# razvanmatisan/duodiff

Measured on AMD Instinct MI355X. Metric: images/sec (whole node) DuoDiff 1000-step CelebA-64, higher is better.
Workload: dtype bf16

## Files before the change

### duodiff_amd/csrc/dev_harness.hip

```cpp
#include "../../include/duodiff.h"
#include "../../include/duodiff_dev.h"
#include "engine_state.h"
#include "launch_args.h"

#include <cstring>
#include <vector>

using namespace dd;

extern "C" {

int dd_dev_mlp(dd_ctx* c, int M, int D, int hidden, int extras, const float* x_host, const float* w1, const float* b1, const float* w2,
               const float* b2, float* xres_host, unsigned short* out_host, const float* ln_in, const float* ln_out,
               unsigned short* ln_out_host, int iters, void* stream, float* ms_out, const float* ao_host, const float* wproj,
               const float* bproj, const float* skip_host, const float* wskip, const float* bskip, const float* wqkv,
               unsigned short* qkv_out_host) {
    const bool proj = ao_host && wproj && bproj;
    const bool skp = skip_host && wskip && bskip;
    const bool qk = wqkv && qkv_out_host;
    if (qk && (!proj || !ln_out || (hidden / 32) % 2)) return DD_ERR_INVALID;
    if (proj && (!ln_in || D % 128)) return DD_ERR_INVALID;
    if (skp && (!proj || !ln_out || !ln_out_host || (hidden / 32) % 2)) return DD_ERR_INVALID;
    if (!c || !x_host || !w1 || !b1 || !w2 || !b2 || !xres_host || M < 1 || iters < 0 || extras < 0 || (extras > 0 && M % (1 + extras))) return DD_ERR_INVALID;
    if (!mlp_fused_supported(D, hidden)) return ctx_fail(c, DD_ERR_UNSUPPORTED, "fused MLP: D in {64,128,256,512}, hidden % 64 == 0");
// ... 506 lines not shown
    const AffineRow* dT = table ? dev.upload(tab.data(), tab.size() * sizeof(AffineRow)) : nullptr;
    const StepState* dS = table ? dev.upload(&st_host, sizeof(StepState)) : nullptr;
    auto once = [&]() { return launch_cache_extrapolate(dL, dP, dO, (long long)n, bf, dS, dT, table ? -1 : op, table ? __builtin_nanf("") : w, s); };
    DEV_HIP(dev, once());
    DEV_HIP(dev, hipStreamSynchronize(s));
    dev.download(out_host, dO, n_out * es);
    DEV_HIP(dev, time_launches(s, iters, once, ms_out));
    return dev.status();
}

int dd_dev_embed(dd_ctx* c, int B, int C, int S, int P, int D, int extras, int num_classes, int normalize, int generic, const float* x_img,
                 const float* w, const float* bias, const float* pos, const float* label_emb, const long long* y, const float* t_vec,
                 float t_state, const float* ln, float* x_tok_host, unsigned short* ln_frag_host, int iters, void* stream, float* ms_out) {
    if (!c || B < 1 || C < 1 || P < 1 || S < P || S % P || D < 2 || extras < 1 || extras > 2 || !x_img || !w || !bias || !pos || !x_tok_host ||
        (extras == 2 && (!label_emb || !y || num_classes < 1)) || (ln && !ln_frag_host) || iters < 0)
        return DD_ERR_INVALID;
    const int pd = C * P * P, L = extras + (S / P) * (S / P), Mp = round_up(B * L, 256);
    if (pd > 64) return ctx_fail(c, DD_ERR_UNSUPPORTED, "embed: patch_dim <= 64");
    hipStream_t s = (hipStream_t)stream;
    const std::vector<float> wt = transposed(w, D, pd);
    const size_t n_tok = ((size_t)Mp + 8) * D;
    EmbedArgs a{};
    a.B = B; a.C = C; a.S = S; a.P = P; a.D = D; a.L = L; a.extras = extras; a.num_classes = num_classes; a.normalize = normalize; a.Mp = Mp;
    a.generic = generic;
    if (ln && !embed_ln_supported(a)) return ctx_fail(c, DD_ERR_UNSUPPORTED, "embed with norm1: the MFMA kernel at patch 4, 3 channels, embed_dim 512");
    DevScope dev(c);
    a.x_img = dev.upload(x_img, (size_t)B * C * S * S * 4);
    a.wt = dev.upload(wt.data(), wt.size() * 4);
    a.bias = dev.upload(bias, (size_t)D * 4);
    a.pos = dev.upload(pos, (size_t)L * D * 4);
    if (extras == 2) { a.label_emb = dev.upload(label_emb, (size_t)num_classes * D * 4); a.y = dev.upload(y, (size_t)B * 8); }
    if (t_vec) a.t_vec = dev.upload(t_vec, (size_t)B * 4);
    a.st = dev.alloc<StepState>(sizeof(StepState));
    a.x_tok = dev.filled<float>(n_tok * 4, 0xFF);
    if (ln) {
        a.ln_g = dev.upload(ln, (size_t)2 * D * 4); a.ln_b = a.ln_g + D;
        a.ln_frag = dev.filled<bf16_t>(n_tok * 2, 0xFF);
    }
    DEV_HIP(dev, launch_set_state_float(a.st, t_state, s));
    auto once = [&]() { return launch_embed(a, s); };
    DEV_HIP(dev, once());
    DEV_HIP(dev, hipStreamSynchronize(s));
    dev.download(x_tok_host, a.x_tok, n_tok * 4);
    if (ln) dev.download(ln_frag_host, a.ln_frag, n_tok * 2);
    DEV_HIP(dev, time_launches(s, iters, once, ms_out));
    return dev.status();
}

int dd_dev_time_mlp(dd_ctx* c, int B, int D, int L, int extras, int normalize, const float* w1, const float* b1, const float* w2,
                    const float* b2, const float* pos, const float* t_vec, float t_state, float* x_tok_host, int iters, void* stream,
                    float* ms_out) {
    if (!c || B < 1 || D < 2 || extras < 1 || L < extras || !w1 || !b1 || !w2 || !b2 || !pos || !x_tok_host || iters < 0) return DD_ERR_INVALID;
    if ((size_t)5 * D * 4 > 64 * 1024) return ctx_fail(c, DD_ERR_UNSUPPORTED, "time_mlp: 5 D floats of LDS");
    hipStream_t s = (hipStream_t)stream;
    const int H4 = 4 * D;
    const std::vector<float> w1t = transposed(w1, H4, D), w2t = transposed(w2, D, H4);
    const size_t n_tok = (size_t)B * L * D;
    DevScope dev(c);
    StepState* st = dev.alloc<StepState>(sizeof(StepState));
    float* dX = dev.upload(x_tok_host, n_tok * 4);
    const TimeMlpArgs a{dev.upload(w1t.data(), w1t.size() * 4), dev.upload(b1, (size_t)H4 * 4), dev.upload(w2t.data(), w2t.size() * 4),
                        dev.upload(b2, (size_t)D * 4), dev.upload(pos, (size_t)L * D * 4), t_vec ? dev.upload(t_vec, (size_t)B * 4) : nullptr,
                        st, dX, B, D, L, extras, normalize};
    DEV_HIP(dev, launch_set_state_float(st, t_state, s));
    auto once = [&]() { return launch_time_mlp(a, s); };
    DEV_HIP(dev, once());
    DEV_HIP(dev, hipStreamSynchronize(s));
    dev.download(x_tok_host, dX, n_tok * 4);
    DEV_HIP(dev, time_launches(s, iters, once, ms_out));
    return dev.status();
}

int dd_dev_vae_gather(dd_ctx* c, int kind, int precision, int B, int H, int W, int Cn, const void* src_host, void* dst_host, size_t dst_bytes,
                      void* stream) {
    const bool bf = precision == DD_PREC_BF16;
    if (!c || (!bf && precision != DD_PREC_FP32) || kind < 0 || kind > 3 || B < 1 || H < 1 || W < 1 || !src_host || !dst_host) return DD_ERR_INVALID;
    if (kind == 3 && (H % 2 || W % 2)) return DD_ERR_INVALID;
// ... 405 lines not shown
```

### duodiff_amd/csrc/mlp_fused.hip

```cpp
#include "dd_internal.h"
#include "wave_prims.h"

#include <type_traits>
#include <utility>

namespace dd {
namespace {

constexpr int kMaxHidden = 4096;
constexpr int kProjRowsLds = 4 * 32 * (1024 + 32);
constexpr int kGroups = 16;

__device__ __forceinline__ const char* uniform_ptr(const char* p) {
    asm volatile("" : "+s"(p));
    return p;
}
__device__ __forceinline__ void glds16u(const char* ubase, unsigned voff, void* lds_dst) {
    __builtin_amdgcn_global_load_lds((gptr_t)(ubase + voff), (lptr_t)lds_dst, 16, 0, 0);
}
template <int J>
__device__ __forceinline__ void glds16u_j(const char* ublock, unsigned voff, char* lds_block) {
    constexpr int HI = (J >> 2) * 4096, IMM = (J & 3) * 1024;
    __builtin_amdgcn_global_load_lds((gptr_t)(ublock + HI + voff), (lptr_t)(lds_block + HI), 16, IMM, 0);
}
// ... 796 lines not shown
    for (int g = 0; g < kGroups; ++g)
        if (g < a.groups) {
#pragma unroll
            for (int e = 0; e < VPL; ++e) acc[e] += pv[g][e];
        }
    float sum = 0.f;
#pragma unroll
    for (int e = 0; e < VPL; ++e) { xv[e] = a.reduce_set ? acc[e] : xv[e] + acc[e]; xp[e] = xv[e]; sum += xv[e]; }
    if (a.y_tap) {
#pragma unroll
        for (int e = 0; e < VPL; ++e) a.y_tap[row * D + col + e] = xv[e];
    }
    if (a.out) {
#pragma unroll
        for (int e = 0; e < VPL; ++e) a.out[row * a.ldo + col + e] = f2bf(xv[e]);
    }
    if (a.ln_out) {
#pragma unroll
        for (int o = 32; o >= 1; o >>= 1) sum += __shfl_xor(sum, o);
        const float mean = sum / (float)D;
        float q2 = 0.f;
#pragma unroll
        for (int e = 0; e < VPL; ++e) { const float d = xv[e] - mean; q2 += d * d; }
#pragma unroll
        for (int o = 32; o >= 1; o >>= 1) q2 += __shfl_xor(q2, o);
        const float rstd = 1.0f / sqrtf(q2 / (float)D + 1e-5f);
#pragma unroll
        for (int e = 0; e < VPL; ++e)
            a.ln_out[row * D + col + e] = f2bf((xv[e] - mean) * rstd * gv[e] + bv[e]);
    }
}

template <int D, int WPG = D / 32, bool LN = true>
__global__ void __launch_bounds__(WPG * 64) skip_rows_ln_kernel(const MlpFusedArgs a) {
    using C = MlpCfg<D>;
    static_assert(!LN || WPG == D / 32, "LayerNorm needs the whole row in one workgroup");
    constexpr int H2 = C::F / 2, PITCH = D * 2 + 16, NW = C::NT, NTHR = WPG * 64;
    extern __shared__ __attribute__((aligned(16))) char srl[];
    char* ybuf = srl;
    char* sbuf = srl + 32 * PITCH;
    float* red = reinterpret_cast<float*>(srl + 64 * PITCH);
    const int tid = threadIdx.x, lane = tid & 63, wave = tid >> 6, h = lane >> 5, r32 = lane & 31;
    auto row_of = [&](int idx) { return extra_token_row(idx, a.n_extra, a.tok_e, a.tok_l); };
    constexpr int CPR = D / 8, ITEMS = 2 * 32 * CPR, PER_ALL = (ITEMS + NTHR - 1) / NTHR, PER = PER_ALL < 8 ? PER_ALL : 8, ROUNDS = (PER_ALL + PER - 1) / PER;
    f32x4 stg[PER];
    auto stage_load = [&](int rd) {
#pragma unroll
        for (int k = 0; k < PER; ++k) {
            const int it = tid + (rd * PER + k) * NTHR, which = it / (32 * CPR), rem = it % (32 * CPR), r = rem / CPR, ch = rem % CPR;
            const long long row = row_of(blockIdx.x * 32 + r);
            const bf16_t* src = which == 0 ? a.out + row * a.ldo : a.skip + row * D;
            stg[k] = it < ITEMS ? *reinterpret_cast<const f32x4*>(src + ch * 8) : f32x4{0.f, 0.f, 0.f, 0.f};
        }
    };
    auto stage_store = [&](int rd) {
#pragma unroll
        for (int k = 0; k < PER; ++k) {
            const int it = tid + (rd * PER + k) * NTHR, which = it / (32 * CPR), rem = it % (32 * CPR), r = rem / CPR, ch = rem % CPR;
            if (it < ITEMS) *reinterpret_cast<f32x4*>((which == 0 ? ybuf : sbuf) + r * PITCH + ch * 16) = stg[k];
        }
    };
    constexpr bool DMA_PARK = !LN && D == 512;
    if constexpr (DMA_PARK) {
#pragma unroll
        for (int i = 0; i < 32 / WPG; ++i) {
            const int r = wave + i * WPG;
            const long long row = row_of(blockIdx.x * 32 + r);
            lds_dma16(a.out + row * a.ldo + lane * 8, ybuf + r * PITCH);
            lds_dma16(a.skip + row * D + lane * 8, sbuf + r * PITCH);
        }
    } else {
        stage_load(0);
    }
    const int t = blockIdx.y * WPG + wave;
    const MlpImage im(D, a.nproj, a.nchunks, a.nskip, a.nqkv);
    const char* const wskip = a.wimg + im.at(im.skip);
    const bf16x8* wy = reinterpret_cast<const bf16x8*>(wskip + (size_t)t * C::BLK) + lane;
    const bf16x8* ws0 = reinterpret_cast<const bf16x8*>(wskip + (size_t)(C::NT + t / 2) * C::BLK) + (t & 1) * H2 * 64 + lane;
    const bf16x8* ws1 = reinterpret_cast<const bf16x8*>(wskip + (size_t)(C::NT + C::NT / 2 + t / 2) * C::BLK) + (t & 1) * H2 * 64 + lane;
    auto wfrag = [&](int kk) -> bf16x8 {
        return kk < C::F ? wy[kk * 64] : kk < C::F + H2 ? ws0[(kk - C::F) * 64] : ws1[(kk - C::F - H2) * 64];
    };
    constexpr int G = 16;
    bf16x8 wf[G];
#pragma unroll
    for (int f = 0; f < G; ++f) wf[f] = wfrag(f);
    if constexpr (DMA_PARK) {
        waitcnt_vm<0>();
    } else {
        stage_store(0);
#pragma unroll
        for (int rd = 1; rd < ROUNDS; ++rd) { stage_load(rd); stage_store(rd); }
    }
    __syncthreads();
    f32x16 acc0, acc1;
#pragma unroll
    for (int g = 0; g < 4; ++g) {
        const f32x4 bq = *reinterpret_cast<const f32x4*>(a.bskip + 32 * t + 8 * g + 4 * h);
#pragma unroll
        for (int e = 0; e < 4; ++e) { acc0[4 * g + e] = bq[e]; acc1[4 * g + e] = 0.f; }
    }
    const char* yrow = ybuf + r32 * PITCH + 8 * h;
    const char* srow = sbuf + r32 * PITCH + 16 * h;
#pragma unroll
    for (int kk = 0; kk < 2 * C::F; ++kk) {
        bf16x8 bfr;
        if (kk < C::F) {
            const u32x2 lo = *reinterpret_cast<const u32x2*>(yrow + 32 * kk), hi = *reinterpret_cast<const u32x2*>(yrow + 32 * kk + 16);
            bfr = __builtin_bit_cast(bf16x8, u32x4{lo[0], lo[1], hi[0], hi[1]});
        } else {
            bfr = *reinterpret_cast<const bf16x8*>(srow + 32 * (kk - C::F));
        }
        if (kk & 1) acc1 = __builtin_amdgcn_mfma_f32_32x32x16_bf16(wf[kk % G], bfr, acc1, 0, 0, 0);
        else acc0 = __builtin_amdgcn_mfma_f32_32x32x16_bf16(wf[kk % G], bfr, acc0, 0, 0, 0);
        if (kk + G < 2 * C::F) wf[kk % G] = wfrag(kk + G);
    }
    const f32x16 acc = acc0 + acc1;
    if constexpr (!LN) {
        const int idx = blockIdx.x * 32 + r32;
        if (idx >= a.n_extra) return;
        const long long row = row_of(idx);
#pragma unroll
        for (int g = 0; g < 4; ++g)
            *reinterpret_cast<f32x4*>(a.xres + row * D + 32 * t + 8 * g + 4 * h) = f32x4{acc[4 * g], acc[4 * g + 1], acc[4 * g + 2], acc[4 * g + 3]};
        return;
    }
    float s1 = 0.f;
#pragma unroll
    for (int e = 0; e < 16; ++e) s1 += acc[e];
    s1 += __shfl_xor(s1, 32);
    if (h == 0) red[wave * 32 + r32] = s1;
    __syncthreads();
    float tot = 0.f;
#pragma unroll
    for (int w = 0; w < NW; ++w) tot += red[w * 32 + r32];
    const float mean = tot / (float)D;
    float s2 = 0.f;
#pragma unroll
    for (int e = 0; e < 16; ++e) { const float d = acc[e] - mean; s2 += d * d; }
    s2 += __shfl_xor(s2, 32);
    if (h == 0) red[(NW + wave) * 32 + r32] = s2;
    __syncthreads();
    float tq = 0.f;
#pragma unroll
    for (int w = 0; w < NW; ++w) tq += red[(NW + w) * 32 + r32];
    const float rstd = 1.0f / sqrtf(tq / (float)D + 1e-5f);
    const int idx = blockIdx.x * 32 + r32;
    if (idx >= a.n_extra) return;
    const long long row = row_of(idx);
// ... 258 lines not shown
```

### duodiff_amd/csrc/rowops.hip

```cpp
#include "dd_internal.h"
#include "wave_prims.h"

#include <cstring>
#include <utility>
#include <vector>

#include <cstdlib>

namespace dd {
namespace {

constexpr int kEmbedTok = 8;

__global__ void __launch_bounds__(256) embed_kernel(const EmbedArgs a) {
    __shared__ float patch[kEmbedTok][64];
    const int rows_per_img_blocks = (a.L + kEmbedTok - 1) / kEmbedTok;
    const int b = blockIdx.x / rows_per_img_blocks;
    const int r0 = (blockIdx.x % rows_per_img_blocks) * kEmbedTok;
    const int tid = threadIdx.x;
    const int pd = a.C * a.P * a.P;
    const int g = a.S / a.P;
    if (blockIdx.x == 0 && tid == 0) a.st->t_final = a.st->t;

    if (b >= a.B) {
// ... 39 lines not shown
            const int row = r0 + j;
            if (row >= a.L) continue;
            float v;
            if (row >= a.extras) {
                v = acc[j] + bias;
            } else if (row == a.extras - 1) {
                const int i = d < halfd ? d : d - halfd;
                const float f = expf((-9.210340371976184f * (float)i) / (float)halfd);
                const float arg = tt * f;
                v = (d < halfd) ? cosf(arg) : (d < 2 * halfd ? sinf(arg) : 0.f);
            } else {
                long long yy = a.y[b];
                yy = yy < 0 ? 0 : (yy >= a.num_classes ? a.num_classes - 1 : yy);
                v = a.label_emb[yy * a.D + d];
            }
            a.x_tok[((long long)b * a.L + row) * a.D + d] = v + a.pos[(long long)row * a.D + d];
        }
    }
}

template <int P, int C, int LND = 0>
__global__ void __launch_bounds__(512) embed_mfma_kernel(const EmbedArgs a) {
    constexpr int PD = P * P * C, KK = PD / 4, KK4 = (KK + 3) / 4;
    static_assert(PD % 4 == 0, "k-steps of 4");
    extern __shared__ __attribute__((aligned(16))) char emb_lds[];
    f32x4* wl = reinterpret_cast<f32x4*>(emb_lds);
    const int tid = threadIdx.x, lane = tid & 63, wave = tid >> 6, n = lane & 15, kq = lane >> 4;
    const int D = a.D, S = a.S, NP = D / 32;
    const int NPY = NP / (int)gridDim.y, p0 = (int)blockIdx.y * NPY;
    const int pass = blockIdx.x * 8 + wave, b = pass >> 4, gy = pass & 15;
    const bool valid = b < a.B;
    if (blockIdx.x == 0 && tid == 0) a.st->t_final = a.st->t;

    float pv[KK];
#pragma unroll
    for (int kk = 0; kk < KK; ++kk) {
        const int k = 4 * kk + kq, c = k / (P * P), p1 = (k / P) % P, p2 = k % P;
        pv[kk] = valid ? a.x_img[(((long long)b * C + c) * S + gy * P + p1) * S + n * P + p2] : 0.f;
    }
    {
        const int items = NPY * 2 * KK4 * 64;
        constexpr int MAXI = 16;
        for (int base = 0; base < items; base += 512 * MAXI) {
            f32x4 v[MAXI];
#pragma unroll
            for (int i = 0; i < MAXI; ++i) {
                const int item = base + tid + 512 * i;
                v[i] = f32x4{0.f, 0.f, 0.f, 0.f};
                if (item < items) {
                    const int l = item & 63, kk4 = (item >> 6) % KK4, ph = (item >> 6) / KK4;
                    const int col = 16 * (ph + 2 * p0) + (l & 15);
#pragma unroll
                    for (int j = 0; j < 4; ++j) {
                        const int kk = 4 * kk4 + j;
                        if (kk < KK) v[i][j] = a.wt[(long long)(4 * kk + (l >> 4)) * D + col];
                    }
                }
            }
#pragma unroll
            for (int i = 0; i < MAXI; ++i) {
                const int item = base + tid + 512 * i;
                if (item < items) wl[item] = v[i];
            }
        }
    }
    __syncthreads();
    if (valid) {
        const long long l0 = a.extras + gy * 16 + n;
        float* xrow = a.x_tok + ((long long)b * a.L + l0) * D + 4 * kq;
        const float* prow = a.pos + l0 * D + 4 * kq;
        const float* brow = a.bias + 4 * kq;
        const f32x4* wlp = wl + lane;
        struct Quads { f32x4 pe, po, be, bo; };
        auto fetch = [&](int pp) -> Quads {
            return Quads{*reinterpret_cast<const f32x4*>(prow + 32 * pp), *reinterpret_cast<const f32x4*>(prow + 32 * pp + 16),
                         *reinterpret_cast<const f32x4*>(brow + 32 * pp), *reinterpret_cast<const f32x4*>(brow + 32 * pp + 16)};
        };
        auto pair = [&](int pp, const Quads& q) {
            f32x4 acc_e = {0.f, 0.f, 0.f, 0.f}, acc_o = {0.f, 0.f, 0.f, 0.f};
#pragma unroll
            for (int kk4 = 0; kk4 < KK4; ++kk4) {
                const f32x4 we = wlp[((2 * (pp - p0)) * KK4 + kk4) * 64], wo = wlp[((2 * (pp - p0) + 1) * KK4 + kk4) * 64];
#pragma unroll
                for (int j = 0; j < 4; ++j) {
                    if (4 * kk4 + j < KK) {
                        acc_e = __builtin_amdgcn_mfma_f32_16x16x4f32(we[j], pv[4 * kk4 + j], acc_e, 0, 0, 0);
                        acc_o = __builtin_amdgcn_mfma_f32_16x16x4f32(wo[j], pv[4 * kk4 + j], acc_o, 0, 0, 0);
                    }
                }
            }
            const f32x4 ve = (acc_e + q.be) + q.pe, vo = (acc_o + q.bo) + q.po;
            *reinterpret_cast<f32x4*>(xrow + 32 * pp) = ve;
            *reinterpret_cast<f32x4*>(xrow + 32 * pp + 16) = vo;
            return std::pair<f32x4, f32x4>{ve, vo};
        };
        Quads qa = fetch(p0), qb = qa;
        if constexpr (LND > 0) {
            constexpr int NPC = LND / 32;
            f32x4 keep[2 * NPC];
#pragma unroll
            for (int p = 0; p < NPC; p += 2) {
                qb = fetch(p + 1);
                const auto r0 = pair(p, qa);
                keep[2 * p] = r0.first; keep[2 * p + 1] = r0.second;
                qa = fetch(p + 2 < NPC ? p + 2 : p + 1);
                const auto r1 = pair(p + 1, qb);
                keep[2 * p + 2] = r1.first; keep[2 * p + 3] = r1.second;
            }
            f32x4 s4 = {0.f, 0.f, 0.f, 0.f};
#pragma unroll
            for (int t = 0; t < 2 * NPC; ++t) s4 += keep[t];
            float sum = (s4[0] + s4[1]) + (s4[2] + s4[3]);
            sum += __shfl_xor(sum, 16);
            sum += __shfl_xor(sum, 32);
            const float mean = sum / (float)LND;
            f32x4 q4 = {0.f, 0.f, 0.f, 0.f};
#pragma unroll
            for (int t = 0; t < 2 * NPC; ++t) { const f32x4 d = keep[t] - mean; q4 += d * d; }
            float q2 = (q4[0] + q4[1]) + (q4[2] + q4[3]);
            q2 += __shfl_xor(q2, 16);
            q2 += __shfl_xor(q2, 32);
            const float rstd = 1.0f / sqrtf(q2 / (float)LND + 1e-5f);
            const long long grp = (long long)b * 8 + (gy >> 1);
            bf16_t* frow = a.ln_frag + ((grp * (LND / 16)) * 64 + ((gy & 1) * 16 + n) + 32 * (kq >> 1)) * 8 + 4 * (kq & 1);
            const float* gr = a.ln_g + 4 * kq;
            const float* br = a.ln_b + 4 * kq;
#pragma unroll
            for (int t = 0; t < 2 * NPC; ++t) {
                const f32x4 gq = *reinterpret_cast<const f32x4*>(gr + 16 * t), bq = *reinterpret_cast<const f32x4*>(br + 16 * t);
                bf16_t o4[4];
#pragma unroll
                for (int e = 0; e < 4; ++e) o4[e] = f2bf((keep[t][e] - mean) * rstd * gq[e] + bq[e]);
                *reinterpret_cast<uint2*>(frow + (long long)t * 512) = *reinterpret_cast<const uint2*>(o4);
            }
        } else {
            for (int p = p0; p < p0 + NPY; p += 2) {
                qb = fetch(p + 1);
                pair(p, qa);
                qa = fetch(p + 2 < p0 + NPY ? p + 2 : p + 1);
                pair(p + 1, qb);
            }
        }
    }
    if (blockIdx.y == 0 && ((blockIdx.x * 8) & 15) == 0 && (int)(blockIdx.x * 8) / 16 < a.B) {
        const int bb = (blockIdx.x * 8) >> 4;
        const float t_raw = a.t_vec ? a.t_vec[bb] : a.st->t_model;
        const float tt = a.normalize ? t_raw / 1000.0f : t_raw;
        const int halfd = D / 2;
        for (int row = 0; row < a.extras; ++row)
            for (int d = tid; d < D; d += 512) {
                float v;
                if (row == a.extras - 1) {
                    const int i = d < halfd ? d : d - halfd;
                    const float arg = tt * expf((-9.210340371976184f * (float)i) / (float)halfd);
                    v = d < halfd ? cosf(arg) : (d < 2 * halfd ? sinf(arg) : 0.f);
                } else {
                    long long yy = a.y[bb];
                    yy = yy < 0 ? 0 : (yy >= a.num_classes ? a.num_classes - 1 : yy);
                    v = a.label_emb[yy * D + d];
                }
                a.x_tok[((long long)bb * a.L + row) * D + d] = v + a.pos[(long long)row * D + d];
            }
    }
    if (blockIdx.x == gridDim.x - 1 && blockIdx.y == 0) {
        const long long first = (long long)a.B * a.L * D, count = ((long long)a.Mp - (long long)a.B * a.L) * D;
        for (long long i = tid; i < count; i += 512) a.x_tok[first + i] = 0.f;
    }
}

__global__ void __launch_bounds__(256) time_mlp_kernel(const TimeMlpArgs a) {
    extern __shared__ float tm_lds[];
    float* e = tm_lds;
    float* hmid = tm_lds + a.D;
    const int b = blockIdx.x, tid = threadIdx.x, D = a.D, H4 = 4 * a.D, halfd = a.D / 2;
    const float t_raw = a.t_vec ? a.t_vec[b] : a.st->t_model;
    const float tt = a.normalize ? t_raw / 1000.0f : t_raw;
    for (int d = tid; d < D; d += 256) {
        const int i = d < halfd ? d : d - halfd;
        const float arg = tt * expf((-9.210340371976184f * (float)i) / (float)halfd);
        e[d] = d < halfd ? cosf(arg) : (d < 2 * halfd ? sinf(arg) : 0.f);
    }
    __syncthreads();
    for (int j = tid; j < H4; j += 256) {
        float acc = a.b1[j];
        for (int k = 0; k < D; ++k) acc = fmaf(a.w1t[(long long)k * H4 + j], e[k], acc);
        hmid[j] = acc / (1.0f + expf(-acc));
    }
    __syncthreads();
    float* row = a.x_tok + ((long long)b * a.L + a.extras - 1) * D;
    for (int d = tid; d < D; d += 256) {
        float acc = a.b2[d];
        for (int k = 0; k < H4; ++k) acc = fmaf(a.w2t[(long long)k * D + d], hmid[k], acc);
        row[d] = acc + a.pos[(long long)(a.extras - 1) * D + d];
    }
}

// ... 224 lines not shown
    }
    __syncthreads();
    float part = 0.f;
    for (int j = tid; j < D; j += 256) {
        float a = w.b0[j];
        for (int k = 0; k < D; ++k) a = fmaf(w.w0t[(long long)k * D + j], ov[k], a);
        hc[j] = a / (1.0f + expf(-a));
        part = fmaf(w.w2[j], hc[j], part);
    }
    part = block_reduce(part, false);
    if (tid == 0) out[b] = part + w.b2[0];
}

}

bool embed_mfma_ok(const EmbedArgs& a, size_t& lds) {
    const int pd = a.C * a.P * a.P;
    lds = (size_t)(a.D / 32) * 2 * ((pd / 4 + 3) / 4) * 1024;
    return a.S == 16 * a.P && a.D % 32 == 0 && pd % 4 == 0 && lds <= 156 * 1024 && a.L == a.extras + 256 &&
           ((a.P == 4 && a.C == 3) || (a.P == 2 && a.C == 3) || (a.P == 2 && a.C == 4));
}

bool embed_ln_supported(const EmbedArgs& a) {
    size_t lds = 0;
    return !a.generic && embed_mfma_ok(a, lds) && a.P == 4 && a.C == 3 && a.D == 512;
}

hipError_t launch_embed(const EmbedArgs& a, hipStream_t s) {
    size_t mlds = 0;
    if (!a.generic && embed_mfma_ok(a, mlds)) {
        dim3 grid((unsigned)((a.B * 16 + 7) / 8));
        if (a.ln_frag) {
            if (!embed_ln_supported(a) || !a.ln_g || !a.ln_b) return hipErrorInvalidValue;
            hipLaunchKernelGGL((embed_mfma_kernel<4, 3, 512>), grid, dim3(512), mlds, s, a);
            return hipGetLastError();
        }
        const int np = a.D / 32;
        while (grid.x * grid.y * 2 <= 256 && np % (grid.y * 4) == 0) grid.y *= 2;
        if (a.P == 4) hipLaunchKernelGGL((embed_mfma_kernel<4, 3>), grid, dim3(512), mlds, s, a);
        else if (a.C == 3) hipLaunchKernelGGL((embed_mfma_kernel<2, 3>), grid, dim3(512), mlds, s, a);
        else hipLaunchKernelGGL((embed_mfma_kernel<2, 4>), grid, dim3(512), mlds, s, a);
        return hipGetLastError();
    }
    const int per_img = (a.L + kEmbedTok - 1) / kEmbedTok;
    const long long pad_rows = (long long)a.Mp - (long long)a.B * a.L;
    const int pad_blocks = (int)((pad_rows + kEmbedTok - 1) / kEmbedTok);
    hipLaunchKernelGGL(embed_kernel, dim3(a.B * per_img + pad_blocks), dim3(256), 0, s, a);
    return hipGetLastError();
}

hipError_t launch_time_mlp(const TimeMlpArgs& a, hipStream_t s) {
    hipLaunchKernelGGL(time_mlp_kernel, dim3(a.B), dim3(256), (size_t)5 * a.D * sizeof(float), s, a);
    return hipGetLastError();
}

template <typename T>
hipError_t launch_layernorm(const float* x, const float* gamma, const float* beta, T* out, int rows,
                            int D, hipStream_t s) {
    if (D % 64 || D > 64 * kLnMaxPerLane) return hipErrorInvalidValue;
    hipLaunchKernelGGL(layernorm_kernel<T>, dim3((rows + 3) / 4), dim3(256), 0, s, x, gamma, beta, out, rows, D, (T*)nullptr, 0, 0);
    return hipGetLastError();
}
hipError_t launch_layernorm_frag(const float* x, const float* gamma, const float* beta, bf16_t* out, bf16_t* frag, int rows, int D,
                                 int tok_l, int tok_e, hipStream_t s) {
    if (D % 256 || D > 64 * kLnMaxPerLane || !frag || tok_l <= tok_e || (tok_l - tok_e) % 32 || rows % tok_l) return hipErrorInvalidValue;
    hipLaunchKernelGGL(layernorm_kernel<bf16_t>, dim3((rows + 3) / 4), dim3(256), 0, s, x, gamma, beta, out, rows, D, frag, tok_l, tok_e);
    return hipGetLastError();
}
hipError_t launch_reduce_ln(const ReduceLnArgs& a, int D, hipStream_t s) {
    if (D % 256 || D > 1024 || a.rows < 1 || a.splits < 1 || !a.x || !a.partial || !a.bias || (a.ln_g && (!a.ln_b || !a.h)) ||
        (a.frag && (a.tok_l <= a.tok_e || (a.tok_l - a.tok_e) % 32 || a.rows % a.tok_l)))
        return hipErrorInvalidValue;
    const dim3 grid((a.rows + 3) / 4);
    switch (D / 256) {
        case 1: hipLaunchKernelGGL(reduce_ln_kernel<1>, grid, dim3(256), 0, s, a); break;
        case 2: hipLaunchKernelGGL(reduce_ln_kernel<2>, grid, dim3(256), 0, s, a); break;
        case 3: hipLaunchKernelGGL(reduce_ln_kernel<3>, grid, dim3(256), 0, s, a); break;
        default: hipLaunchKernelGGL(reduce_ln_kernel<4>, grid, dim3(256), 0, s, a); break;
    }
    return hipGetLastError();
}
template hipError_t launch_layernorm<bf16_t>(const float*, const float*, const float*, bf16_t*, int, int, hipStream_t);
template hipError_t launch_layernorm<float>(const float*, const float*, const float*, float*, int, int, hipStream_t);

template <int OFF, bool HAND>
__device__ __forceinline__ void asm_load_quad(f32x4& dst, const float* p) {
    if constexpr (HAND) asm volatile("global_load_dwordx4 %0, %1, off offset:%2" : "=v"(dst) : "v"(p), "i"(OFF));
    else dst = *reinterpret_cast<const f32x4*>(p + OFF / 4);
}
template <int N, bool HAND>
__device__ __forceinline__ void landed_at_vmcnt(f32x4& v) {
    static_assert(!HAND || N < 64, "a 6-bit counter");
    if constexpr (HAND) asm volatile("s_waitcnt vmcnt(%1)" : "+v"(v) : "n"(N));
}

template <int D, int NT, int NW = 8, bool PROBE = false, bool SPLIT = false>
__global__ void __launch_bounds__(NW * 64) head_dec_kernel(const HeadDecArgs a) {
    constexpr int J = D / 16;
    constexpr auto quad_off = [](int jq) constexpr { return SPLIT ? 128 * (jq / 2) + 16 * (jq % 2) : 64 * jq; };
    constexpr int KG = SPLIT ? 8 : 4;
    constexpr bool HAND = J + J * NT / NW + (PROBE ? 1 : 0) <= 52;
    extern __shared__ __attribute__((aligned(16))) char head_lds[];
    f32x4* wl = reinterpret_cast<f32x4*>(head_lds);
    f32x4* pwl = wl + J * NT * 64;
    const int lane = threadIdx.x & 63, wave = threadIdx.x >> 6, n = lane & 15, q = lane >> 4;
    static_assert(!PROBE || (D % 256 == 0 && D / 256 <= NW), "the probe row is staged by D / 256 waves");
    int pi = 0;
    if constexpr (PROBE) pi = (a.t_mul ? a.st->t_final * a.t_mul : 0) + a.add;
    const int upi = a.tok_l > 0 ? (a.tok_l - a.tok_e) / 16 : 0;
    const int units = a.tok_l > 0 ? (a.M / a.tok_l) * upi : (a.M + 15) / 16, stride = NW * (int)gridDim.x;
    auto row_of = [&](int u) -> long long {
        return a.tok_l > 0 ? (long long)(u / upi) * a.tok_l + a.tok_e + (u % upi) * 16 + n : (long long)u * 16 + n;
    };
    f32x4 xv[J];
    auto request = [&](int u) {
        const long long row = row_of(u);
        const float* xr = a.x + (row < a.M ? row : (long long)a.M - 1) * D + KG * q;
        [&]<int... JJ>(std::integer_sequence<int, JJ...>) {
            (asm_load_quad<quad_off(JJ), HAND>(xv[JJ], xr), ...);
        }(std::make_integer_sequence<int, J>{});
    };
    constexpr int WI = J * NT / NW;
    static_assert(J * NT % NW == 0, "one equal share of Wg fragments per wave");
    static_assert(quad_off(J - 1) < 4096, "the row quads' immediate offsets");
    static_assert(!SPLIT || (HAND && J % 2 == 0), "the split product is built for the hand-counted widths");
    static_assert(!HAND || J + WI <= 63, "the vector-memory counter holds 63 operations");
    int u = wave * (int)gridDim.x + (int)blockIdx.x;
// ... 266 lines not shown
```

### duodiff_amd/csrc/wave_prims.h

```cpp
#pragma once
#include "dd_internal.h"

namespace dd {

typedef const __attribute__((address_space(1))) void* gptr_t;
typedef __attribute__((address_space(3))) void* lptr_t;

__device__ __forceinline__ unsigned cvt_pk_bf16(float lo, float hi) {
    typedef __bf16 bf16v2 __attribute__((ext_vector_type(2)));
    typedef float f32v2 __attribute__((ext_vector_type(2)));
    const f32v2 q = {lo, hi};
    return __builtin_bit_cast(unsigned, __builtin_convertvector(q, bf16v2));
}

__device__ __forceinline__ unsigned lds_offset(const void* p) { return (unsigned)(size_t)(const __attribute__((address_space(3))) char*)p; }

__device__ __forceinline__ void lds_dma16(const void* src, void* lds_dst) {
    __builtin_amdgcn_global_load_lds((gptr_t)src, (lptr_t)lds_dst, 16, 0, 0);
}
__device__ __forceinline__ void lds_dma16s(const char* sbase, unsigned voff, const void* lds_dst) {
    asm volatile("s_mov_b32 m0, %0\n\ts_nop 0\n\tglobal_load_lds_dwordx4 %1, %2" ::"s"(lds_offset(lds_dst)), "v"(voff), "s"(sbase) : "memory", "m0");
}

template <int N>
__device__ __forceinline__ void waitcnt_vm() { asm volatile("s_waitcnt vmcnt(%0)" ::"i"(N) : "memory"); }

template <int OFF, typename V>
__device__ __forceinline__ void ds_read16(V& dst, unsigned addr) {
    static_assert(sizeof(V) == 16, "one ds_read_b128");
    asm volatile("ds_read_b128 %0, %1 offset:%2" : "=v"(dst) : "v"(addr), "i"(OFF));
}

#define DD_S_MFMA_W "s_waitcnt lgkmcnt(%[lg])\n\tv_mfma_f32_32x32x16_bf16 %[acc], %[wa], %[xb], %[acc]"
#define DD_S_MFMA_N "v_mfma_f32_32x32x16_bf16 %[acc], %[wa], %[xb], %[acc]"
#define DD_S_READ "\n\tds_read_b128 %[wa], %[la] offset:%[lo]"
#define DD_MFMA_GAP(ACC_C)                                                                                                                                \
    if constexpr (LG >= 0) {                                                                                                                              \
        if constexpr (READ) asm volatile(DD_S_MFMA_W DD_S_READ : [acc] ACC_C(acc), [wa] "+v"(wa) : [xb] "v"(xb), [la] "v"(la), [lg] "i"(LG), [lo] "i"(LO)); \
        else asm volatile(DD_S_MFMA_W : [acc] ACC_C(acc), [wa] "+v"(wa) : [xb] "v"(xb), [lg] "i"(LG));                                                    \
    } else {                                                                                                                                              \
        if constexpr (READ) asm volatile(DD_S_MFMA_N DD_S_READ : [acc] ACC_C(acc), [wa] "+v"(wa) : [xb] "v"(xb), [la] "v"(la), [lo] "i"(LO));              \
        else asm volatile(DD_S_MFMA_N : [acc] ACC_C(acc), [wa] "+v"(wa) : [xb] "v"(xb));                                                                  \
    }
template <bool AGPR, int LG, bool READ, int LO>
__device__ __forceinline__ void mfma_gap(f32x16& acc, bf16x8& wa, const bf16x8& xb, unsigned la) {
    if constexpr (AGPR) { DD_MFMA_GAP("+a") } else { DD_MFMA_GAP("+v") }
}
#undef DD_MFMA_GAP

__device__ __forceinline__ float wave_reduce_add(float v) {
#pragma unroll
    for (int o = 32; o >= 1; o >>= 1) v += __shfl_xor(v, o);
    return v;
}

__device__ __forceinline__ long long extra_token_row(int idx, int n_extra, int tok_e, int tok_l) {
    const int q = idx < n_extra ? idx : n_extra - 1, b = q / tok_e;
    return (long long)b * tok_l + (q - b * tok_e);
// ... 4 lines not shown
```

Baseline: 50.39.

## Prefetch weights and positional rows with hand-counted vmcnt loads in skip and embed kernels

The skip-rows kernel now issues its bias and weight fragment loads as inline-asm global loads and waits on exact vmcnt values per MFMA step, so the weight stream stays in flight across the fully unrolled K loop. It also asks for two waves per EU. The embed kernel with LayerNorm prefetches the positional rows into registers before the LDS staging and stages bias, gamma and beta in LDS, which removes global loads from the post-barrier compute path. It computes the extra tokens before the barrier. The harness gains canary rows to check that the embed kernel does not write out of bounds. These changes raise register pressure and depend on fragile hand-tracked counters.

```diff
diff --git a/duodiff_amd/csrc/dev_harness.hip b/duodiff_amd/csrc/dev_harness.hip
--- a/duodiff_amd/csrc/dev_harness.hip
+++ b/duodiff_amd/csrc/dev_harness.hip
@@ -562,10 +562,14 @@
     if (extras == 2) { a.label_emb = dev.upload(label_emb, (size_t)num_classes * D * 4); a.y = dev.upload(y, (size_t)B * 8); }
     if (t_vec) a.t_vec = dev.upload(t_vec, (size_t)B * 4);
     a.st = dev.alloc<StepState>(sizeof(StepState));
-    a.x_tok = dev.filled<float>(n_tok * 4, 0xFF);
+    const size_t guard = (size_t)8 * D;
+    float* x_buf = dev.filled<float>((guard + n_tok) * 4, 0xFF);
+    bf16_t* f_buf = nullptr;
+    a.x_tok = x_buf ? x_buf + guard : nullptr;
     if (ln) {
         a.ln_g = dev.upload(ln, (size_t)2 * D * 4); a.ln_b = a.ln_g + D;
-        a.ln_frag = dev.filled<bf16_t>(n_tok * 2, 0xFF);
+        f_buf = dev.filled<bf16_t>((guard + n_tok) * 2, 0xFF);
+        a.ln_frag = f_buf ? f_buf + guard : nullptr;
     }
     DEV_HIP(dev, launch_set_state_float(a.st, t_state, s));
     auto once = [&]() { return launch_embed(a, s); };
@@ -573,6 +577,12 @@
     DEV_HIP(dev, hipStreamSynchronize(s));
     dev.download(x_tok_host, a.x_tok, n_tok * 4);
     if (ln) dev.download(ln_frag_host, a.ln_frag, n_tok * 2);
+    std::vector<unsigned char> front(guard * 6, 0xFF);
+    dev.download(front.data(), x_buf, guard * 4);
+    if (ln) dev.download(front.data() + guard * 4, f_buf, guard * 2);
+    if (!dev.ok()) return dev.status();
+    for (unsigned char v : front)
+        if (v != 0xFF) return ctx_fail(c, DD_ERR_STATE, "embed: the canary rows in front of x_tok or ln_frag were written");
     DEV_HIP(dev, time_launches(s, iters, once, ms_out));
     return dev.status();
 }
diff --git a/duodiff_amd/csrc/mlp_fused.hip b/duodiff_amd/csrc/mlp_fused.hip
--- a/duodiff_amd/csrc/mlp_fused.hip
+++ b/duodiff_amd/csrc/mlp_fused.hip
@@ -852,7 +852,7 @@
 }
 
 template <int D, int WPG = D / 32, bool LN = true>
-__global__ void __launch_bounds__(WPG * 64) skip_rows_ln_kernel(const MlpFusedArgs a) {
+__global__ void __launch_bounds__(WPG * 64) __attribute__((amdgpu_waves_per_eu(2))) skip_rows_ln_kernel(const MlpFusedArgs a) {
     using C = MlpCfg<D>;
     static_assert(!LN || WPG == D / 32, "LayerNorm needs the whole row in one workgroup");
     constexpr int H2 = C::F / 2, PITCH = D * 2 + 16, NW = C::NT, NTHR = WPG * 64;
@@ -898,13 +898,22 @@
     const bf16x8* wy = reinterpret_cast<const bf16x8*>(wskip + (size_t)t * C::BLK) + lane;
     const bf16x8* ws0 = reinterpret_cast<const bf16x8*>(wskip + (size_t)(C::NT + t / 2) * C::BLK) + (t & 1) * H2 * 64 + lane;
     const bf16x8* ws1 = reinterpret_cast<const bf16x8*>(wskip + (size_t)(C::NT + C::NT / 2 + t / 2) * C::BLK) + (t & 1) * H2 * 64 + lane;
-    auto wfrag = [&](int kk) -> bf16x8 {
-        return kk < C::F ? wy[kk * 64] : kk < C::F + H2 ? ws0[(kk - C::F) * 64] : ws1[(kk - C::F - H2) * 64];
+    constexpr int NK = 2 * C::F;
+    constexpr int G = NTHR > 512 ? 8 : 16;
+    static_assert(H2 % 4 == 0 && NK >= G, "whole groups of four fragments per weight block");
+    auto wreq = [&]<int KK>(std::integral_constant<int, KK>, f32x4& dst) {
+        constexpr int g4 = KK & ~3;
+        const bf16x8* base = g4 < C::F ? wy + g4 * 64 : g4 < C::F + H2 ? ws0 + (g4 - C::F) * 64 : ws1 + (g4 - C::F - H2) * 64;
+        asm_load_quad<(KK & 3) * 1024, true>(dst, reinterpret_cast<const float*>(base));
     };
-    constexpr int G = 16;
-    bf16x8 wf[G];
-#pragma unroll
-    for (int f = 0; f < G; ++f) wf[f] = wfrag(f);
+    f32x4 bq[4], wf[G];
+    {
+        const float* bp = a.bskip + 32 * t + 4 * h;
+        [&]<int... GI>(std::integer_sequence<int, GI...>) {
+            (asm_load_quad<32 * GI, true>(bq[GI], bp), ...);
+        }(std::make_integer_sequence<int, 4>{});
+    }
+    [&]<int... FI>(std::integer_sequence<int, FI...>) { (wreq(std::integral_constant<int, FI>{}, wf[FI]), ...); }(std::make_integer_sequence<int, G>{});
     if constexpr (DMA_PARK) {
         waitcnt_vm<0>();
     } else {
@@ -916,25 +925,29 @@
     f32x16 acc0, acc1;
 #pragma unroll
     for (int g = 0; g < 4; ++g) {
-        const f32x4 bq = *reinterpret_cast<const f32x4*>(a.bskip + 32 * t + 8 * g + 4 * h);
-#pragma unroll
-        for (int e = 0; e < 4; ++e) { acc0[4 * g + e] = bq[e]; acc1[4 * g + e] = 0.f; }
+        landed_at_vmcnt<G, true>(bq[g]);
+#pragma unroll
+        for (int e = 0; e < 4; ++e) { acc0[4 * g + e] = bq[g][e]; acc1[4 * g + e] = 0.f; }
     }
     const char* yrow = ybuf + r32 * PITCH + 8 * h;
     const char* srow = sbuf + r32 * PITCH + 16 * h;
-#pragma unroll
-    for (int kk = 0; kk < 2 * C::F; ++kk) {
-        bf16x8 bfr;
-        if (kk < C::F) {
-            const u32x2 lo = *reinterpret_cast<const u32x2*>(yrow + 32 * kk), hi = *reinterpret_cast<const u32x2*>(yrow + 32 * kk + 16);
-            bfr = __builtin_bit_cast(bf16x8, u32x4{lo[0], lo[1], hi[0], hi[1]});
-        } else {
-            bfr = *reinterpret_cast<const bf16x8*>(srow + 32 * (kk - C::F));
-        }
-        if (kk & 1) acc1 = __builtin_amdgcn_mfma_f32_32x32x16_bf16(wf[kk % G], bfr, acc1, 0, 0, 0);
-        else acc0 = __builtin_amdgcn_mfma_f32_32x32x16_bf16(wf[kk % G], bfr, acc0, 0, 0, 0);
-        if (kk + G < 2 * C::F) wf[kk % G] = wfrag(kk + G);
-    }
+    [&]<int... KK>(std::integer_sequence<int, KK...>) {
+        ([&] {
+            constexpr int kk = KK;
+            bf16x8 bfr;
+            if constexpr (kk < C::F) {
+                const u32x2 lo = *reinterpret_cast<const u32x2*>(yrow + 32 * kk), hi = *reinterpret_cast<const u32x2*>(yrow + 32 * kk + 16);
+                bfr = __builtin_bit_cast(bf16x8, u32x4{lo[0], lo[1], hi[0], hi[1]});
+            } else {
+                bfr = *reinterpret_cast<const bf16x8*>(srow + 32 * (kk - C::F));
+            }
+            landed_at_vmcnt<(NK - kk < G ? NK - kk : G) - 1, true>(wf[kk % G]);
+            if constexpr (kk & 1) acc1 = __builtin_amdgcn_mfma_f32_32x32x16_bf16(__builtin_bit_cast(bf16x8, wf[kk % G]), bfr, acc1, 0, 0, 0);
+            else acc0 = __builtin_amdgcn_mfma_f32_32x32x16_bf16(__builtin_bit_cast(bf16x8, wf[kk % G]), bfr, acc0, 0, 0, 0);
+            if constexpr (kk + G < NK) wreq(std::integral_constant<int, kk + G>{}, wf[kk % G]);
+        }(), ...);
+    }(std::make_integer_sequence<int, NK>{});
+    asm volatile("" : "+v"(acc0), "+v"(acc1));
     const f32x16 acc = acc0 + acc1;
     if constexpr (!LN) {
         const int idx = blockIdx.x * 32 + r32;
diff --git a/duodiff_amd/csrc/rowops.hip b/duodiff_amd/csrc/rowops.hip
--- a/duodiff_amd/csrc/rowops.hip
+++ b/duodiff_amd/csrc/rowops.hip
@@ -95,6 +95,14 @@
     const bool valid = b < a.B;
     if (blockIdx.x == 0 && tid == 0) a.st->t_final = a.st->t;
 
+    constexpr int NQ = LND > 0 ? LND / 16 : 1;
+    f32x4 keep[NQ];
+    if constexpr (LND > 0) {
+        static_assert(64 * (NQ - 1) < 4096 && NQ <= 32, "the quads' immediate offsets; pos -> keep is half the wave's registers");
+        const float* prow = a.pos + (long long)(a.extras + gy * 16 + n) * LND + 4 * kq;
+        [&]<int... T>(std::integer_sequence<int, T...>) { (asm_load_quad<64 * T, true>(keep[T], prow), ...); }(std::make_integer_sequence<int, NQ>{});
+    }
+
     float pv[KK];
 #pragma unroll
     for (int kk = 0; kk < KK; ++kk) {
@@ -104,6 +112,13 @@
     {
         const int items = NPY * 2 * KK4 * 64;
         constexpr int MAXI = 16;
+        f32x4 vq = {0.f, 0.f, 0.f, 0.f};
+        if constexpr (LND > 0) {
+            static_assert(3 * LND / 4 <= 512, "one quad of the vectors per thread");
+            const int vi = tid < 3 * LND / 4 ? tid : 0;
+            const float* src = vi < LND / 4 ? a.bias + 4 * vi : vi < LND / 2 ? a.ln_g + 4 * (vi - LND / 4) : a.ln_b + 4 * (vi - LND / 2);
+            vq = *reinterpret_cast<const f32x4*>(src);
+        }
         for (int base = 0; base < items; base += 512 * MAXI) {
             f32x4 v[MAXI];
 #pragma unroll
@@ -126,86 +141,12 @@
                 if (item < items) wl[item] = v[i];
             }
         }
-    }
-    __syncthreads();
-    if (valid) {
-        const long long l0 = a.extras + gy * 16 + n;
-        float* xrow = a.x_tok + ((long long)b * a.L + l0) * D + 4 * kq;
-        const float* prow = a.pos + l0 * D + 4 * kq;
-        const float* brow = a.bias + 4 * kq;
-        const f32x4* wlp = wl + lane;
-        struct Quads { f32x4 pe, po, be, bo; };
-        auto fetch = [&](int pp) -> Quads {
-            return Quads{*reinterpret_cast<const f32x4*>(prow + 32 * pp), *reinterpret_cast<const f32x4*>(prow + 32 * pp + 16),
-                         *reinterpret_cast<const f32x4*>(brow + 32 * pp), *reinterpret_cast<const f32x4*>(brow + 32 * pp + 16)};
-        };
-        auto pair = [&](int pp, const Quads& q) {
-            f32x4 acc_e = {0.f, 0.f, 0.f, 0.f}, acc_o = {0.f, 0.f, 0.f, 0.f};
-#pragma unroll
-            for (int kk4 = 0; kk4 < KK4; ++kk4) {
-                const f32x4 we = wlp[((2 * (pp - p0)) * KK4 + kk4) * 64], wo = wlp[((2 * (pp - p0) + 1) * KK4 + kk4) * 64];
-#pragma unroll
-                for (int j = 0; j < 4; ++j) {
-                    if (4 * kk4 + j < KK) {
-                        acc_e = __builtin_amdgcn_mfma_f32_16x16x4f32(we[j], pv[4 * kk4 + j], acc_e, 0, 0, 0);
-                        acc_o = __builtin_amdgcn_mfma_f32_16x16x4f32(wo[j], pv[4 * kk4 + j], acc_o, 0, 0, 0);
-                    }
-                }
-            }
-            const f32x4 ve = (acc_e + q.be) + q.pe, vo = (acc_o + q.bo) + q.po;
-            *reinterpret_cast<f32x4*>(xrow + 32 * pp) = ve;
-            *reinterpret_cast<f32x4*>(xrow + 32 * pp + 16) = vo;
-            return std::pair<f32x4, f32x4>{ve, vo};
-        };
-        Quads qa = fetch(p0), qb = qa;
         if constexpr (LND > 0) {
-            constexpr int NPC = LND / 32;
-            f32x4 keep[2 * NPC];
-#pragma unroll
-            for (int p = 0; p < NPC; p += 2) {
-                qb = fetch(p + 1);
-                const auto r0 = pair(p, qa);
-                keep[2 * p] = r0.first; keep[2 * p + 1] = r0.second;
-                qa = fetch(p + 2 < NPC ? p + 2 : p + 1);
-                const auto r1 = pair(p + 1, qb);
-                keep[2 * p + 2] = r1.first; keep[2 * p + 3] = r1.second;
-            }
-            f32x4 s4 = {0.f, 0.f, 0.f, 0.f};
-#pragma unroll
-            for (int t = 0; t < 2 * NPC; ++t) s4 += keep[t];
-            float sum = (s4[0] + s4[1]) + (s4[2] + s4[3]);
-            sum += __shfl_xor(sum, 16);
-            sum += __shfl_xor(sum, 32);
-            const float mean = sum / (float)LND;
-            f32x4 q4 = {0.f, 0.f, 0.f, 0.f};
-#pragma unroll
-            for (int t = 0; t < 2 * NPC; ++t) { const f32x4 d = keep[t] - mean; q4 += d * d; }
-            float q2 = (q4[0] + q4[1]) + (q4[2] + q4[3]);
-            q2 += __shfl_xor(q2, 16);
-            q2 += __shfl_xor(q2, 32);
-            const float rstd = 1.0f / sqrtf(q2 / (float)LND + 1e-5f);
-            const long long grp = (long long)b * 8 + (gy >> 1);
-            bf16_t* frow = a.ln_frag + ((grp * (LND / 16)) * 64 + ((gy & 1) * 16 + n) + 32 * (kq >> 1)) * 8 + 4 * (kq & 1);
-            const float* gr = a.ln_g + 4 * kq;
-            const float* br = a.ln_b + 4 * kq;
-#pragma unroll
-            for (int t = 0; t < 2 * NPC; ++t) {
-                const f32x4 gq = *reinterpret_cast<const f32x4*>(gr + 16 * t), bq = *reinterpret_cast<const f32x4*>(br + 16 * t);
-                bf16_t o4[4];
-#pragma unroll
-                for (int e = 0; e < 4; ++e) o4[e] = f2bf((keep[t][e] - mean) * rstd * gq[e] + bq[e]);
-                *reinterpret_cast<uint2*>(frow + (long long)t * 512) = *reinterpret_cast<const uint2*>(o4);
-            }
-        } else {
-            for (int p = p0; p < p0 + NPY; p += 2) {
-                qb = fetch(p + 1);
-                pair(p, qa);
-                qa = fetch(p + 2 < p0 + NPY ? p + 2 : p + 1);
-                pair(p + 1, qb);
-            }
-        }
-    }
-    if (blockIdx.y == 0 && ((blockIdx.x * 8) & 15) == 0 && (int)(blockIdx.x * 8) / 16 < a.B) {
+            if (tid < 3 * LND / 4) wl[items + tid] = vq;
+        }
+    }
+    auto extra_tokens = [&]() {
+        if (!(blockIdx.y == 0 && ((blockIdx.x * 8) & 15) == 0 && (int)(blockIdx.x * 8) / 16 < a.B)) return;
         const int bb = (blockIdx.x * 8) >> 4;
         const float t_raw = a.t_vec ? a.t_vec[bb] : a.st->t_model;
         const float tt = a.normalize ? t_raw / 1000.0f : t_raw;
@@ -224,7 +165,100 @@
                 }
                 a.x_tok[((long long)bb * a.L + row) * D + d] = v + a.pos[(long long)row * D + d];
             }
-    }
+    };
+    if constexpr (LND > 0) {
+        [&]<int... T>(std::integer_sequence<int, T...>) { (landed_at_vmcnt<NQ - 1 - T, true>(keep[T]), ...); }(std::make_integer_sequence<int, NQ>{});
+        extra_tokens();
+    }
+    __syncthreads();
+    if constexpr (LND > 0) {
+        if (valid) {
+            constexpr int NPC = LND / 32;
+            const f32x4* wlp = wl + lane;
+            const f32x4* vecs = wl + NPC * 2 * KK4 * 64 + kq;
+            float* xrow = a.x_tok + ((long long)b * a.L + a.extras + gy * 16 + n) * LND + 4 * kq;
+#pragma unroll
+            for (int p = 0; p < NPC; ++p) {
+                f32x4 acc_e = {0.f, 0.f, 0.f, 0.f}, acc_o = {0.f, 0.f, 0.f, 0.f};
+#pragma unroll
+                for (int kk4 = 0; kk4 < KK4; ++kk4) {
+                    const f32x4 we = wlp[((2 * p) * KK4 + kk4) * 64], wo = wlp[((2 * p + 1) * KK4 + kk4) * 64];
+#pragma unroll
+                    for (int j = 0; j < 4; ++j) {
+                        if (4 * kk4 + j < KK) {
+                            acc_e = __builtin_amdgcn_mfma_f32_16x16x4f32(we[j], pv[4 * kk4 + j], acc_e, 0, 0, 0);
+                            acc_o = __builtin_amdgcn_mfma_f32_16x16x4f32(wo[j], pv[4 * kk4 + j], acc_o, 0, 0, 0);
+                        }
+                    }
+                }
+                keep[2 * p] = (acc_e + vecs[8 * p]) + keep[2 * p];
+                keep[2 * p + 1] = (acc_o + vecs[8 * p + 4]) + keep[2 * p + 1];
+                *reinterpret_cast<f32x4*>(xrow + 32 * p) = keep[2 * p];
+                *reinterpret_cast<f32x4*>(xrow + 32 * p + 16) = keep[2 * p + 1];
+                __builtin_amdgcn_sched_barrier(0);
+            }
+            f32x4 s4 = {0.f, 0.f, 0.f, 0.f};
+#pragma unroll
+            for (int t = 0; t < 2 * NPC; ++t) s4 += keep[t];
+            float sum = (s4[0] + s4[1]) + (s4[2] + s4[3]);
+            sum += __shfl_xor(sum, 16);
+            sum += __shfl_xor(sum, 32);
+            const float mean = sum / (float)LND;
+            f32x4 q4 = {0.f, 0.f, 0.f, 0.f};
+#pragma unroll
+            for (int t = 0; t < 2 * NPC; ++t) { const f32x4 d = keep[t] - mean; q4 += d * d; }
+            float q2 = (q4[0] + q4[1]) + (q4[2] + q4[3]);
+            q2 += __shfl_xor(q2, 16);
+            q2 += __shfl_xor(q2, 32);
+            const float rstd = 1.0f / sqrtf(q2 / (float)LND + 1e-5f);
+            const long long grp = (long long)b * 8 + (gy >> 1);
+            bf16_t* frow = a.ln_frag + ((grp * (LND / 16)) * 64 + ((gy & 1) * 16 + n) + 32 * (kq >> 1)) * 8 + 4 * (kq & 1);
+#pragma unroll
+            for (int t = 0; t < 2 * NPC; ++t) {
+                const f32x4 gq = vecs[LND / 4 + 4 * t], bq = vecs[LND / 2 + 4 * t];
+                bf16_t o4[4];
+#pragma unroll
+                for (int e = 0; e < 4; ++e) o4[e] = f2bf((keep[t][e] - mean) * rstd * gq[e] + bq[e]);
+                *reinterpret_cast<uint2*>(frow + (long long)t * 512) = *reinterpret_cast<const uint2*>(o4);
+            }
+        }
+    } else if (valid) {
+        const long long l0 = a.extras + gy * 16 + n;
+        float* xrow = a.x_tok + ((long long)b * a.L + l0) * D + 4 * kq;
+        const float* prow = a.pos + l0 * D + 4 * kq;
+        const float* brow = a.bias + 4 * kq;
+        const f32x4* wlp = wl + lane;
+        struct Quads { f32x4 pe, po, be, bo; };
+        auto fetch = [&](int pp) -> Quads {
+            return Quads{*reinterpret_cast<const f32x4*>(prow + 32 * pp), *reinterpret_cast<const f32x4*>(prow + 32 * pp + 16),
+                         *reinterpret_cast<const f32x4*>(brow + 32 * pp), *reinterpret_cast<const f32x4*>(brow + 32 * pp + 16)};
+        };
+        auto pair = [&](int pp, const Quads& q) {
+            f32x4 acc_e = {0.f, 0.f, 0.f, 0.f}, acc_o = {0.f, 0.f, 0.f, 0.f};
+#pragma unroll
+            for (int kk4 = 0; kk4 < KK4; ++kk4) {
+                const f32x4 we = wlp[((2 * (pp - p0)) * KK4 + kk4) * 64], wo = wlp[((2 * (pp - p0) + 1) * KK4 + kk4) * 64];
+#pragma unroll
+                for (int j = 0; j < 4; ++j) {
+                    if (4 * kk4 + j < KK) {
+                        acc_e = __builtin_amdgcn_mfma_f32_16x16x4f32(we[j], pv[4 * kk4 + j], acc_e, 0, 0, 0);
+                        acc_o = __builtin_amdgcn_mfma_f32_16x16x4f32(wo[j], pv[4 * kk4 + j], acc_o, 0, 0, 0);
+                    }
+                }
+            }
+            const f32x4 ve = (acc_e + q.be) + q.pe, vo = (acc_o + q.bo) + q.po;
+            *reinterpret_cast<f32x4*>(xrow + 32 * pp) = ve;
+            *reinterpret_cast<f32x4*>(xrow + 32 * pp + 16) = vo;
+        };
+        Quads qa = fetch(p0), qb = qa;
+        for (int p = p0; p < p0 + NPY; p += 2) {
+            qb = fetch(p + 1);
+            pair(p, qa);
+            qa = fetch(p + 2 < p0 + NPY ? p + 2 : p + 1);
+            pair(p + 1, qb);
+        }
+    }
+    if constexpr (LND == 0) extra_tokens();
     if (blockIdx.x == gridDim.x - 1 && blockIdx.y == 0) {
         const long long first = (long long)a.B * a.L * D, count = ((long long)a.Mp - (long long)a.B * a.L) * D;
         for (long long i = tid; i < count; i += 512) a.x_tok[first + i] = 0.f;
@@ -515,7 +549,7 @@
         dim3 grid((unsigned)((a.B * 16 + 7) / 8));
         if (a.ln_frag) {
             if (!embed_ln_supported(a) || !a.ln_g || !a.ln_b) return hipErrorInvalidValue;
-            hipLaunchKernelGGL((embed_mfma_kernel<4, 3, 512>), grid, dim3(512), mlds, s, a);
+            hipLaunchKernelGGL((embed_mfma_kernel<4, 3, 512>), grid, dim3(512), mlds + 3 * 512 * sizeof(float), s, a);
             return hipGetLastError();
         }
         const int np = a.D / 32;
@@ -565,17 +599,6 @@
 }
 template hipError_t launch_layernorm<bf16_t>(const float*, const float*, const float*, bf16_t*, int, int, hipStream_t);
 template hipError_t launch_layernorm<float>(const float*, const float*, const float*, float*, int, int, hipStream_t);
-
-template <int OFF, bool HAND>
-__device__ __forceinline__ void asm_load_quad(f32x4& dst, const float* p) {
-    if constexpr (HAND) asm volatile("global_load_dwordx4 %0, %1, off offset:%2" : "=v"(dst) : "v"(p), "i"(OFF));
-    else dst = *reinterpret_cast<const f32x4*>(p + OFF / 4);
-}
-template <int N, bool HAND>
-__device__ __forceinline__ void landed_at_vmcnt(f32x4& v) {
-    static_assert(!HAND || N < 64, "a 6-bit counter");
-    if constexpr (HAND) asm volatile("s_waitcnt vmcnt(%1)" : "+v"(v) : "n"(N));
-}
 
 template <int D, int NT, int NW = 8, bool PROBE = false, bool SPLIT = false>
 __global__ void __launch_bounds__(NW * 64) head_dec_kernel(const HeadDecArgs a) {
diff --git a/duodiff_amd/csrc/wave_prims.h b/duodiff_amd/csrc/wave_prims.h
--- a/duodiff_amd/csrc/wave_prims.h
+++ b/duodiff_amd/csrc/wave_prims.h
@@ -24,6 +24,17 @@
 
 template <int N>
 __device__ __forceinline__ void waitcnt_vm() { asm volatile("s_waitcnt vmcnt(%0)" ::"i"(N) : "memory"); }
+
+template <int OFF, bool HAND>
+__device__ __forceinline__ void asm_load_quad(f32x4& dst, const float* p) {
+    if constexpr (HAND) asm volatile("global_load_dwordx4 %0, %1, off offset:%2" : "=v"(dst) : "v"(p), "i"(OFF));
+    else dst = *reinterpret_cast<const f32x4*>(p + OFF / 4);
+}
+template <int N, bool HAND>
+__device__ __forceinline__ void landed_at_vmcnt(f32x4& v) {
+    static_assert(!HAND || N < 64, "a 6-bit counter");
+    if constexpr (HAND) asm volatile("s_waitcnt vmcnt(%1)" : "+v"(v) : "n"(N));
+}
 
 template <int OFF, typename V>
 __device__ __forceinline__ void ds_read16(V& dst, unsigned addr) {
```

Measured after the change: 50.73 (median of 3 runs). No clear change (+0.7%).
